# Onetism/LightFieldMicroscopy_PC-bzip2

Measured on AMD Instinct MI355X. Metric: uint16 Mpixel/s encode (predictor->bzip2) at 1/2/4/8 GPUs; ratio parity, higher is better.
Workload: dtype u16

## Files before the change

### include/lfm/lfm_hip.h

```cpp
#ifndef LFM_HIP_H
#define LFM_HIP_H

#include <stdint.h>
#include <stddef.h>

#ifdef __cplusplus
extern "C" {
#endif

enum lfm_hip_status {
    LFM_HIP_OK = 0,
    LFM_HIP_EINVAL = 1,
    LFM_HIP_ERUNTIME = 2,
    LFM_HIP_ENOTINV = 3,
    LFM_HIP_ENODEV = 4
};


int lfm_hip_predict(const uint16_t* d_in, const uint16_t* d_prev, uint16_t* d_out, int W, int H, int nframes,
                    int T, int family, int predictor, int video_bit, int z0, void* stream);

int lfm_hip_unpredict(const uint16_t* d_sym, const uint16_t* d_prev, uint16_t* d_out, int W, int H, int nframes,
                      int T, int family, int predictor, int video_bit, int z0, void* stream);
int lfm_hip_unpredict_async(const uint16_t* d_sym, const uint16_t* d_prev, uint16_t* d_out, int W, int H,
// ... 3 lines not shown
int lfm_hip_unpredict_path(int W, int H, int T);

int lfm_hip_predict_candidates(const uint16_t* d_frame, uint16_t* d_out7, int W, int H, int T, int family,
                               void* stream);

int lfm_hip_entropy2d(const uint16_t* d_cand, uint64_t npix, float* entropy, void* stream);

size_t lfm_hip_select_workspace_bytes(int W, int H);
int lfm_hip_select(const uint16_t* d_frame, int W, int H, int T, int family, float entropy[8], int* chosen,
                   void* d_workspace, void* stream);

size_t lfm_hip_bzip2_workspace_bytes(uint32_t count, uint32_t block_bytes);
size_t lfm_hip_bzip2_out_cap(uint32_t block_bytes);
int lfm_hip_bzip2_blocks(const void* d_img, const uint32_t dims[5], const uint32_t bs[5], uint32_t bpp,
                         uint32_t first, uint32_t count, uint32_t level, void* d_ws, size_t ws_bytes,
                         void* d_payload, uint64_t* h_sizes, uint32_t* h_flags, void* stream);
size_t lfm_hip_bzip2_workspace_bytes_multi(uint32_t count, uint32_t block_bytes, uint32_t level);
uint32_t lfm_hip_bzip2_max_count_multi(uint32_t block_bytes, uint32_t level);
int lfm_hip_bzip2_blocks_multi(const void* d_img, const uint32_t dims[5], const uint32_t bs[5], uint32_t bpp,
                               uint32_t first, uint32_t count, uint32_t level, void* d_ws, size_t ws_bytes,
                               void* d_payload, uint64_t* h_sizes, uint32_t* h_flags, void* stream);
uint64_t lfm_hip_bzip2_last_blocks(void);
void lfm_hip_bzip2_last_bwt_stats(uint32_t out[12]);
int lfm_hip_bzip2_last_stage_ms(float ms[5]);
void lfm_hip_bzip2_set_stage_hook(void (*fn)(void* ctx, int stage), void* ctx);

size_t lfm_hip_bunzip2_workspace_bytes(uint32_t count, uint32_t out_stride);
int lfm_hip_bunzip2_blocks(const void* d_payload, const uint64_t* h_offs, uint32_t count, void* d_out,
                           uint32_t out_stride, void* d_ws, size_t ws_bytes, uint32_t* h_lens, uint32_t* h_flags,
                           void* stream);
int lfm_hip_bunzip2_issue(const void* d_payload, const uint64_t* h_offs, uint32_t count, void* d_out,
                          uint32_t out_stride, void* d_ws, size_t ws_bytes, uint32_t* h_lens, uint32_t* h_flags,
                          void* stream);
uint32_t lfm_hip_bunzip2_max_parts(uint32_t out_stride, uint32_t level);
size_t lfm_hip_bunzip2_workspace_bytes_multi(uint32_t count, uint32_t out_stride, uint32_t level);
int lfm_hip_bunzip2_blocks_multi(const void* d_payload, const uint64_t* h_offs, uint32_t count, void* d_out,
                                 uint32_t out_stride, uint32_t level, void* d_ws, size_t ws_bytes, uint32_t* h_lens,
                                 uint32_t* h_flags, void* stream);
int lfm_hip_bunzip2_issue_multi(const void* d_payload, const uint64_t* h_offs, uint32_t count, void* d_out,
                                uint32_t out_stride, uint32_t level, void* d_ws, size_t ws_bytes, uint32_t* h_lens,
                                uint32_t* h_flags, void* stream);
int lfm_hip_bunzip2_set_periodic(int on);
int lfm_hip_bunzip2_get_periodic(void);

int lfm_hip_scatter_blocks(const void* d_blocks, uint32_t stride, uint32_t first, uint32_t count,
                           const uint32_t dims[5], const uint32_t bs[5], uint32_t bpp, void* d_img, void* stream);
// ... 16 lines not shown
```

### lightfieldmicroscopy_pc-bzip2_amd/csrc/lfm_bzip2.hip

```cpp
#include <hip/hip_runtime.h>
#include <rocprim/block/block_exchange.hpp>
#include <rocprim/block/block_sort.hpp>
#include <rocprim/device/device_radix_sort.hpp>
#include <rocprim/device/device_scan.hpp>
#include <rocprim/device/device_segmented_radix_sort.hpp>
#include <rocprim/device/device_select.hpp>
#include <rocprim/iterator/counting_iterator.hpp>
#include <algorithm>
#include <climits>
#include <cstdlib>
#include <cstdint>
#include <cstdio>
#include <cstring>
#include <mutex>
#include <type_traits>
#include <vector>
#include "lfm_bwt_types.h"
#include "lfm_bz_caps.h"
#include "lfm_hip.h"

#ifndef LFM_BWT_FORCE_FULL
#define LFM_BWT_FORCE_FULL 0
#endif

// ... 1012 lines not shown
            continue;
        }
        uint32_t* sv = B.sa + slot;
        bool ok = true;
        for (uint32_t x = 1; x < g && ok; ++x) {
            const uint32_t vx = sv[x];
            uint32_t y = x;
            while (y > 0) {
                const int cmp = tie_cmp(T, n, sv[y - 1] & kIdxMask, vx & kIdxMask);
                if (cmp == 0) {
                    ok = false;
                    break;
                }
                if (cmp < 0) break;
                sv[y] = sv[y - 1];
                --y;
            }
            sv[y] = vx;
        }
        if (!ok) atomicAdd(unres, 1u);
    }
}

template <int TH, int IPT>
__device__ __forceinline__ void chunk_load(const Batch& B, uint32_t cb, uint32_t m, uint32_t t, uint64_t (&k)[IPT],
                                           uint32_t (&v)[IPT])
{
    const uint32_t s = cb / B.cap, n = B.n[s];
    const uint8_t* T = B.T + (size_t)s * B.cap;
#pragma unroll
    for (int q = 0; q < IPT; ++q) v[q] = B.vals_a[cb + min(q * TH + t, m ? m - 1u : 0u)];
    uint32_t d[IPT][3];
#pragma unroll
    for (int q = 0; q < IPT; ++q) {
        const uint32_t i = v[q] & kIdxMask;
        const uint32_t* w = (const uint32_t*)(T + ((i + 8u <= n ? i : 0u) & ~3u));
        d[q][0] = w[0];
        d[q][1] = w[1];
        d[q][2] = w[2];
    }
#pragma unroll
    for (int q = 0; q < IPT; ++q) {
        const uint32_t j = q * TH + t, i = v[q] & kIdxMask;
        if (j >= m) {
            k[q] = ~0ull;
            v[q] = 0u;
        } else if (i + 8u <= n) {
            const uint32_t sh = (i & 3u) * 8u;
            const uint64_t x = (uint64_t)d[q][0] | ((uint64_t)d[q][1] << 32);
            k[q] = __builtin_bswap64(sh ? (x >> sh) | ((uint64_t)d[q][2] << (64u - sh)) : x);
        } else {
            k[q] = rot_key8_fast(T, n, i);
        }
    }
}

template <int TH, int IPT>
__global__ __launch_bounds__(TH) void bwt_chunk_sort(Batch B, const uint32_t* __restrict__ cbp,
                                                     const uint32_t* __restrict__ cep, uint32_t nch, uint32_t per)
{
    const uint32_t c = per ? (blockIdx.x & 7u) * per + (blockIdx.x >> 3) : blockIdx.x;
    if (c >= nch) return;
    static_assert(IPT == 2 || IPT == 4 || IPT == 8, "flags are packed 2, 4 or 8 per thread");
    using Sort = rocprim::block_sort<uint64_t, TH, IPT, uint32_t, rocprim::block_sort_algorithm::merge_sort>;
    using ExK = rocprim::block_exchange<uint64_t, TH, IPT>;
    using ExV = rocprim::block_exchange<uint32_t, TH, IPT>;
    constexpr uint32_t NI = TH * IPT;
    struct Xch {
        uint64_t first[TH], last[TH];
        uint32_t sv[NI];
        uint8_t fl[NI];
    };
    __shared__ union alignas(16) {
        typename Sort::storage_type s;
        typename ExK::storage_type ek;
        typename ExV::storage_type ev;
        Xch x;
    } sm;
    const uint32_t cb = cbp[c], ce = cep[c], m = ce - cb, t = threadIdx.x;
    uint64_t k[IPT];
    uint32_t v[IPT];
    chunk_load<TH, IPT>(B, cb, m, t, k, v);
    ExK().striped_to_blocked(k, k, sm.ek);
    __syncthreads();
    ExV().striped_to_blocked(v, v, sm.ev);
    __syncthreads();
    Sort().sort(k, v, sm.s, m);
    __syncthreads();
    sm.x.first[t] = k[0];
    sm.x.last[t] = k[IPT - 1];
    __syncthreads();
    const uint64_t kprev = t ? sm.x.last[t - 1] : 0ull, knext = t + 1 < (uint32_t)TH ? sm.x.first[t + 1] : 0ull;
    uint32_t nt = 0;
    uint64_t fpack = 0;
#pragma unroll
    for (int q = 0; q < IPT; ++q) {
        const uint32_t pos = t * IPT + q;
        const uint64_t lo = q ? k[q - 1] : kprev, hi = q + 1 < IPT ? k[q + 1] : knext;
        const bool f = pos < m && ((pos > 0 && lo == k[q]) || (pos + 1 < m && hi == k[q]));
        nt += f ? 1u : 0u;
        fpack |= (uint64_t)(f ? 1u : 0u) << (8 * q);
    }
    if constexpr (IPT == 2) {
        *(uint2*)&sm.x.sv[t * IPT] = make_uint2(v[0], v[1]);
        *(uint16_t*)&sm.x.fl[t * IPT] = (uint16_t)fpack;
    } else {
#pragma unroll
        for (int q = 0; q < IPT; q += 4) *(uint4*)&sm.x.sv[t * IPT + q] = make_uint4(v[q], v[q + 1], v[q + 2], v[q + 3]);
        if constexpr (IPT == 8) *(uint64_t*)&sm.x.fl[t * IPT] = fpack;
        else *(uint32_t*)&sm.x.fl[t * IPT] = (uint32_t)fpack;
    }
    __syncthreads();
    for (uint32_t j = t; j < m; j += TH) {
        B.sa[cb + j] = sm.x.sv[j];
        B.uflag[cb + j] = sm.x.fl[j];
    }
    if (__any(nt)) {
        for (int d = 32; d > 0; d >>= 1) nt += __shfl_xor(nt, d);
        if ((threadIdx.x & 63) == 0 && nt) atomicAdd(&B.done[cb / B.cap], nt);
    }
}

__device__ __forceinline__ uint64_t rot_key8(const Batch& B, uint32_t s, uint32_t i)
{
    const uint32_t n = B.n[s];
    const uint8_t* T = B.T + (size_t)s * B.cap;
    uint64_t k = 0;
    uint32_t j = i;
#pragma unroll
    for (int q = 0; q < 8; ++q) {
        k = (k << 8) | T[j];
        j = j + 1 == n ? 0u : j + 1;
    }
    return k;
}

__device__ __forceinline__ uint8_t tied_flag(const uint64_t* __restrict__ K, uint32_t cb, uint32_t ce, uint32_t j,
                                             uint64_t k)
// ... 238 lines not shown
__global__ __launch_bounds__(256) void bwt_comp_rank(Batch B, const uint32_t* __restrict__ cnt_p,
                                                     const uint32_t* __restrict__ hvs)
{
    const uint32_t cnt = *cnt_p;
    for (uint32_t c = blockIdx.x * blockDim.x + threadIdx.x; c < cnt; c += gridDim.x * blockDim.x) {
        const uint32_t head_slot = hvs[c];
        const uint32_t s = head_slot / B.cap;
        const size_t o = (size_t)s * B.cap;
        B.rank[o + (B.vals_b[c] & kIdxMask)] = (uint32_t)(head_slot - o);
        const bool head = c == 0 || B.keys_b[c] != B.keys_b[c - 1];
        const bool next_head = c + 1 >= cnt || B.keys_b[c + 1] != B.keys_b[c];
        B.uflag[c] = (head && next_head) ? 0 : 1;
    }
}

__global__ __launch_bounds__(256) void bwt_flag_periodic(Batch B, const uint32_t* __restrict__ cl,
                                                         const uint32_t* __restrict__ cnt_p)
{
    const uint32_t cnt = *cnt_p;
    for (uint32_t c = blockIdx.x * blockDim.x + threadIdx.x; c < cnt; c += gridDim.x * blockDim.x)
        atomicOr(&B.flags[cl[c] / B.cap], kFlagHost);
}

__device__ __forceinline__ void make_u2s(const Batch& B, uint32_t s, uint8_t* u2s, uint32_t lane, uint32_t* nin_out)
{
    uint32_t inu[8], nin = 0;
#pragma unroll
    for (int q = 0; q < 8; ++q) {
        inu[q] = B.inuse[s * 8 + q];
        nin += __popc(inu[q]);
    }
    for (uint32_t c = lane; c < 256; c += 64) {
        uint32_t below = 0;
        for (uint32_t q = 0; q < (c >> 5); ++q) below += __popc(inu[q]);
        below += __popc(inu[c >> 5] & ((1u << (c & 31)) - 1u));
        u2s[c] = (uint8_t)below;
    }
    *nin_out = nin;
}

constexpr uint32_t kIndPend = 0xFFFFFFFFu;
constexpr uint32_t kIndIdx = 0xFFFFFu;
constexpr uint32_t kIndPlaced = 1u << 23;
constexpr uint32_t kPlaceChunk = 2048;

__global__ __launch_bounds__(256) void bwt_place_sorted(Batch B, uint32_t chunks)
{
    __shared__ uint32_t tq[256], cs[256], cl[256], s0[256];
    __shared__ uint32_t cb[256];
    __shared__ uint8_t u2s[256];
    const uint32_t t = threadIdx.x, k = blockIdx.x >> 3;
    const uint32_t s = (blockIdx.x & 7u) + 8u * (k / chunks), base = (k % chunks) * kPlaceChunk;
    if (s >= B.nstreams || (B.flags[s] & kFlagHost)) return;
    const uint32_t n = B.n[s], ns = B.nsub[s], mode = B.bwt_mode[s];
    if (base >= n) return;
    const bool rev = mode == kModeSortA;
    if (t < 64) {
        uint32_t nin;
        make_u2s(B, s, u2s, t, &nin);
    }
    {
        const uint32_t* it = B.itab + (size_t)s * 1024;
        const uint32_t u = rev ? 255u - t : t;
        tq[t] = it[t];
        cs[t] = it[256 + t];
        cl[t] = it[512 + t];
        s0[t] = it[768 + t];
        cb[t] = it[256 + u] + it[512 + u] + (rev ? B.abcnt[(size_t)s * 512 + t] - 1u : 0u);
    }
    __syncthreads();
    const size_t o = (size_t)s * B.cap;
    const uint8_t* T = B.T + o;
    uint8_t* LL = (uint8_t*)B.mtfv + o;
    uint2* E = B.ent + o;
    constexpr int K = kPlaceChunk / 256;
    uint32_t v[K], w0[K], w1[K];
#pragma unroll
    for (int q = 0; q < K; ++q) v[q] = B.sa[o + min(base + q * 256 + t, ns ? ns - 1 : 0u)];
#pragma unroll
    for (int q = 0; q < K; ++q) {
        const uint32_t i = v[q] & kIdxMask, a = i >= 4 ? i - 4 : 0u;
        const uint32_t* w = (const uint32_t*)(T + (a & ~3u));
        w0[q] = w[0];
        w1[q] = w[1];
    }
#pragma unroll
    for (int q = 0; q < K; ++q) {
        const uint32_t j = base + q * 256 + t;
        if (j >= ns) break;
        const uint32_t i = v[q] & kIdxMask;
        uint32_t x;
        uint32_t c;
        if (i >= 4) {
            const uint32_t sh = ((i - 4) & 3u) * 8u;
            const uint64_t d = (uint64_t)w0[q] | ((uint64_t)w1[q] << 32);
            x = (uint32_t)(d >> sh);
            c = (uint32_t)(d >> (sh + 32)) & 0xFFu;
        } else {
            x = 0;
            for (uint32_t r = 1; r <= 4; ++r) x |= (uint32_t)T[(i + 4 * n - r) % n] << (32 - 8 * r);
            c = T[i];
        }
        const uint32_t r = j - s0[c], qq = tq[c] + r;
        LL[qq] = u2s[v[q] >> 24];
        if (i == 0) B.orig_ptr[s] = qq;
        if (mode != kModeFull)
            E[rev ? cb[c] - r : cb[c] + r] =
                make_uint2(v[q] | (3u << 20),
                           ((x >> 16) & 0xFFu) | (((x >> 8) & 0xFFu) << 8) | ((x & 0xFFu) << 16) | (c << 24));
    }
    if (mode == kModeFull) return;
    const uint32_t end = base + kPlaceChunk;
    uint32_t lo = 0, hi = 255;
    while (lo < hi) {
        const uint32_t mid = (lo + hi + 1) >> 1;
        if (cs[mid] <= base) lo = mid;
        else hi = mid - 1;
    }
    for (uint32_t u = lo; u < 256 && cs[u] < end; ++u)
        for (uint32_t q = max(cs[u], base) + t; q < min(cs[u] + cl[u], end); q += 256) E[q] = make_uint2(kIndPend, 0u);
}

constexpr uint32_t kIndSlices = 8;
constexpr uint32_t kIndBlock = 64 * kIndSlices;
constexpr int kIndStepSlices = 4;
constexpr uint32_t kIndRing = 2 * kIndBlock;

__device__ __forceinline__ void glds16(const void* g, const void* lds)
{
    const uint32_t m0 = __builtin_amdgcn_readfirstlane(
        (uint32_t)(size_t)(const __attribute__((address_space(3))) void*)lds);
    asm volatile("s_mov_b32 m0, %0\n\ts_nop 0\n\tglobal_load_lds_dwordx4 %1, off sc1" ::"s"(m0), "v"(g) : "memory", "m0");
}

__device__ __forceinline__ void vm_drain() { asm volatile("s_waitcnt vmcnt(0)" ::: "memory"); }

__global__ __launch_bounds__(64) void bwt_induce(Batch B)
{
    __shared__ uint32_t head[256], hlim[256];
    __shared__ uint32_t chead[256], clim[256];
    __shared__ uint2 ring[kIndRing];
    __shared__ __attribute__((aligned(16))) uint2 stg[kIndBlock];
    __shared__ uint8_t u2s[256];
// ... 1621 lines not shown
    float last_ms[5] = {};
    bool valid = false;
    ~StageEvents()
    {
        for (hipEvent_t e : ev)
            if (e) (void)hipEventDestroy(e);
    }
    bool ready(int d)
    {
        if (dev == d) return true;
        for (hipEvent_t& e : ev) {
            if (e) (void)hipEventDestroy(e);
            e = nullptr;
            if (hipEventCreate(&e) != hipSuccess) return false;
        }
        dev = d;
        return true;
    }
};
thread_local StageEvents t_stage;
thread_local void (*t_hook)(void*, int) = nullptr;
thread_local void* t_hook_ctx = nullptr;
thread_local uint64_t t_last_blocks = 0;
thread_local uint32_t t_last_bwt[12] = {};

size_t prim_tmp_bytes(uint32_t count, uint32_t cap)
{
    const size_t N = (size_t)count * cap;
    uint64_t* k = nullptr;
    uint32_t* v = nullptr;
    uint8_t* f = nullptr;
    size_t tmp = 0, q = 0;
    const size_t max_seg = (size_t)count * (cap / kBigCap + 1);
    (void)rocprim::segmented_radix_sort_pairs(nullptr, q, k, k, v, v, (unsigned)N, (unsigned)max_seg, v, v, 0,
                                              64 - kBucketBits);
    tmp = std::max(tmp, q);
    (void)rocprim::radix_sort_pairs(nullptr, q, k, k, v, v, (unsigned)N, 0, 64);
    tmp = std::max(tmp, q);

    (void)rocprim::select(nullptr, q, rocprim::counting_iterator<uint32_t>(0), f, v, v, N);
    tmp = std::max(tmp, q);
    (void)rocprim::select(nullptr, q, v, f, v, v, N);
    tmp = std::max(tmp, q);
    (void)rocprim::inclusive_scan(nullptr, q, v, v, N, rocprim::maximum<uint32_t>());
    tmp = std::max(tmp, q);
    return tmp;
}

struct Scratch {
    uint64_t* offs;
    uint32_t* cnt;
    void* tmp;
    size_t tmp_bytes;
};

struct BwtStats {
    uint32_t chunks[4] = {};
    uint32_t first_ties = 0;
    uint32_t left_runs = 0;
    uint32_t text_rounds = 0;
    uint32_t restarted = 0;
    uint32_t rank_form = 0;
    uint32_t doubling_rounds = 0;
    uint32_t flag_periodic = 0;
};

size_t layout(uint8_t* base, uint32_t streams, uint32_t block_bytes, uint32_t level, Batch& B, Scratch& S)
{
    B.parts = level ? max_parts(block_bytes, level) : 1u;
    const uint32_t count = streams * B.parts;
    B.nstreams = count;
    B.raw_cap = (uint32_t)align_up(block_bytes, 16);
    B.cap = rle_cap(block_bytes);
    B.out_cap = out_cap(block_bytes);
    B.sel_cap = sel_cap(block_bytes);
    B.full_cap = B.cap;
    if (B.parts > 1) {
        const uint32_t part_max = 100000u * level - 19u + 5u;
        B.cap = std::min(B.cap, (uint32_t)align_up((size_t)part_max + 64, 256));
        B.out_cap = std::min(B.out_cap, out_cap(part_max));
        B.sel_cap = (uint32_t)align_up(B.cap / kGSize + 8, 64);
    }
    B.jcap = B.parts * B.out_cap;
    B.pay_cap = out_cap(block_bytes);
    const size_t n = count, N = n * B.cap;
    size_t off = 0;
    auto take = [&](auto*& p, size_t bytes) {
// ... 47 lines not shown
struct TieRounds {
    hipStream_t st;
    size_t N;
    uint32_t* cnt;
    void* tmp;
    size_t tmp_bytes;
    uint32_t* cl;
    uint32_t* cl_next;
    uint32_t covered;
    bool none_left;
    BwtStats stats;
    uint64_t* gk;

    hipError_t read_count(uint32_t* out, size_t bytes = 4)
    {
        hipError_t e = hipMemcpyAsync(out, cnt, bytes, hipMemcpyDeviceToHost, st);
        return e != hipSuccess ? e : hipStreamSynchronize(st);
    }
};

uint32_t list_grid(uint32_t cnt) { return std::min<uint32_t>(4096, (cnt + 255) / 256); }

template <int TH, int IPT>
void chunk_sorts(const Batch& B, const ChunkLists& CL, int cls, uint32_t nc, hipStream_t st)
{
    const uint32_t per = (nc + 7) / 8;
    if (nc) hipLaunchKernelGGL((bwt_chunk_sort<TH, IPT>), dim3(8 * per), dim3(TH), 0, st, B, CL.b[cls], CL.e[cls], nc, per);
}

hipError_t first_round(const Batch& B, TieRounds& W)
{
    hipStream_t st = W.st;
    const uint32_t count = B.nstreams;
    hipError_t e;
    ChunkLists CL;
    const size_t q = W.N / 4;
    for (int c = 0; c < 4; ++c) {
        CL.b[c] = B.cl0 + c * q;
        CL.e[c] = B.cl1 + c * q;
    }
    CL.cnt = W.cnt;
    CL.cnt3 = W.cnt + 5;
    uint32_t nch[6] = {0, 0, 0, 0, 0, 0};
    if ((e = hipMemsetAsync(W.cnt, 0, 32, st)) != hipSuccess ||
        (e = hipMemsetAsync(B.done, 0, (size_t)count * 4, st)) != hipSuccess)
        return e;
    hipLaunchKernelGGL(bwt_bucket<kBucketBits>, dim3(count), dim3(kBucketThreads), 0, st, B, CL);
    if ((e = hipGetLastError()) != hipSuccess || (e = W.read_count(nch, 24)) != hipSuccess) return e;
    W.stats.chunks[0] = nch[5];
    W.stats.chunks[1] = nch[0];
    W.stats.chunks[2] = nch[1];
    W.stats.chunks[3] = nch[2];
    W.stats.first_ties = W.stats.left_runs = W.stats.text_rounds = 0;
    chunk_sorts<kTinyCap / kCsItems, kCsItems>(B, CL, 3, nch[5], st);
    chunk_sorts<kCsThreads, kCsItems>(B, CL, 0, nch[0], st);
    chunk_sorts<kBigThreads, kBigItems>(B, CL, 1, nch[1], st);
    if (nch[2]) {
        hipLaunchKernelGGL(bwt_chunk_keys, dim3(nch[2]), dim3(256), 0, st, B, CL.b[2], CL.e[2]);
        e = rocprim::segmented_radix_sort_pairs(W.tmp, W.tmp_bytes, B.keys_a, B.keys_b, B.vals_a, B.sa,
                                                (unsigned)W.N, nch[2], CL.b[2], CL.e[2], 0, 64 - kBucketBits, st);
        if (e == hipSuccess)
            hipLaunchKernelGGL(bwt_chunk_flags, dim3(nch[2]), dim3(256), 0, st, B, CL.b[2], CL.e[2]);
    }
    if ((e = hipGetLastError()) != hipSuccess) return e;
    W.cl = B.cl0;
    W.cl_next = B.cl1;
    hipLaunchKernelGGL(tie_offsets, dim3(1), dim3(1024), 0, st, B, W.cnt);
    hipLaunchKernelGGL(tie_compact, dim3(count), dim3(256), 0, st, B, B.cl0);
    hipLaunchKernelGGL(tie_runs_direct, dim3(1024), dim3(256), 0, st, B, B.cl0, W.cnt, W.cnt + 7);
    W.covered = kKeyBytes;
    W.none_left = false;
    return hipGetLastError();
}

hipError_t text_rounds(const Batch& B, TieRounds& W)
{
    hipStream_t st = W.st;
    uint32_t* bnd = (uint32_t*)B.mtfv;
    for (int r = 0; r < kTextRounds; ++r) {
        uint32_t c8[8] = {};
        hipError_t e = W.read_count(c8, r == 0 ? 32 : 4);
        if (e != hipSuccess) return e;
        const uint32_t cnt = c8[0];
        if (r == 0) {
            W.stats.first_ties = cnt;
            W.stats.left_runs = c8[7];
        }
        if (cnt == 0 || (r == 0 && c8[7] == 0)) {
            W.none_left = true;
            break;
        }
        if ((size_t)cnt * 4 > W.N) break;
// ... 168 lines not shown
    Scratch S{};
    if (ws_bytes < layout((uint8_t*)d_ws, streams, raw_cap, multi ? level : 0u, B, S)) return LFM_HIP_EINVAL;
    count = B.nstreams;
    if ((size_t)count * B.cap >= (1ull << 32)) return LFM_HIP_EINVAL;
    const bool parts = B.parts > 1;

    hipError_t e = hipSuccess;
    auto ok = [&]() { return (e = hipGetLastError()) == hipSuccess; };
    const bool from_img = ((uintptr_t)d_img & 15) == 0 && (bs[0] * bpp) % 16 == 0 && (dims[0] * bpp) % 16 == 0 &&
                          ((dims[0] % bs[0]) * bpp) % 16 == 0;
    mark(0);
    if (!from_img) hipLaunchKernelGGL(gather_blocks, dim3(64, streams), dim3(256), 0, st, B);
    if (!parts) {
        if (from_img) hipLaunchKernelGGL((rle1_crc<true, false>), dim3(count), dim3(kRleThreads), 0, st, B);
        else hipLaunchKernelGGL((rle1_crc<false, false>), dim3(count), dim3(kRleThreads), 0, st, B);
    } else {
        if (from_img) hipLaunchKernelGGL((rle1_crc<true, true>), dim3(streams), dim3(kRleThreads), 0, st, B);
        else hipLaunchKernelGGL((rle1_crc<false, true>), dim3(streams), dim3(kRleThreads), 0, st, B);
        hipLaunchKernelGGL(place_parts, dim3(16, count), dim3(256), 0, st, B);
    }
    if (!ok()) return LFM_HIP_ERUNTIME;
    mark(1);
    BwtStats bwt_stats;
    if (bwt_sort(B, S, st, &bwt_stats) != hipSuccess) return LFM_HIP_ERUNTIME;
    {
        const uint32_t v[12] = {bwt_stats.chunks[0], bwt_stats.chunks[1], bwt_stats.chunks[2], bwt_stats.chunks[3],
                                bwt_stats.first_ties, bwt_stats.left_runs, bwt_stats.text_rounds, bwt_stats.restarted,
                                bwt_stats.rank_form, bwt_stats.doubling_rounds, bwt_stats.flag_periodic, 0u};
        std::copy(v, v + 12, t_last_bwt);
    }
    if (!B.it_full) {
        B.ent = (uint2*)B.keys_a;
        const uint32_t chunks = (B.cap + kPlaceChunk - 1) / kPlaceChunk;
        hipLaunchKernelGGL(bwt_place_sorted, dim3(8 * chunks * ((count + 7) / 8)), dim3(256), 0, st, B, chunks);
        hipLaunchKernelGGL(bwt_induce, dim3(count), dim3(64), 0, st, B);
        if (!ok()) return LFM_HIP_ERUNTIME;
    }
    mark(2);
    if (t_hook) t_hook(t_hook_ctx, 1);
    {
        const uint32_t nseg_max = (B.cap + kSeg - 1) / kSeg;
        int32_t* seg_last = (int32_t*)B.keys_a;
        const dim3 g((nseg_max + 3) / 4, count);
        if (B.it_full) hipLaunchKernelGGL(mtf_last<false>, g, dim3(256), 0, st, B, nseg_max, seg_last);
        else hipLaunchKernelGGL(mtf_last<true>, g, dim3(256), 0, st, B, nseg_max, seg_last);
        hipLaunchKernelGGL(mtf_prefix, dim3(count), dim3(256), 0, st, B, nseg_max, seg_last);
        hipLaunchKernelGGL(mtf_win, g, dim3(256), 0, st, B, nseg_max, (const int32_t*)seg_last);
        hipLaunchKernelGGL(rle2, dim3(count), dim3(kRle2Threads), 0, st, B);
    }
    uint32_t nwide = 0;
    if (!ok() || hipMemcpyAsync(&nwide, B.wide_cnt, 4, hipMemcpyDeviceToHost, st) != hipSuccess ||
        hipStreamSynchronize(st) != hipSuccess || nwide > count)
        return LFM_HIP_ERUNTIME;
    mark(3);
    if (t_hook) t_hook(t_hook_ctx, 2);
    hipLaunchKernelGGL(huff_init, dim3(count), dim3(64), 0, st, B);
    static thread_local struct TablesEvent {
// ... 73 lines not shown

extern "C" int lfm_hip_bzip2_blocks_multi(const void* d_img, const uint32_t dims[5], const uint32_t bs[5],
                                          uint32_t bpp, uint32_t first, uint32_t count, uint32_t level, void* d_ws,
                                          size_t ws_bytes, void* d_payload, uint64_t* h_sizes, uint32_t* h_flags,
                                          void* stream)
{
    return bzip2_blocks(d_img, dims, bs, bpp, first, count, level, d_ws, ws_bytes, d_payload, h_sizes, h_flags, stream,
                        true);
}

extern "C" void lfm_hip_bzip2_set_stage_hook(void (*fn)(void*, int), void* ctx)
{
    t_hook = fn;
    t_hook_ctx = ctx;
}

extern "C" uint64_t lfm_hip_bzip2_last_blocks(void) { return t_last_blocks; }

extern "C" void lfm_hip_bzip2_last_bwt_stats(uint32_t out[12])
{
    if (out) std::copy(t_last_bwt, t_last_bwt + 12, out);
}

extern "C" int lfm_hip_bzip2_last_stage_ms(float ms[5])
{
    if (!ms || !t_stage.valid) return 3;
    for (int i = 0; i < 5; ++i) ms[i] = t_stage.last_ms[i];
    return 0;
}
```

### lightfieldmicroscopy_pc-bzip2_amd/lfm/__init__.py

```python
import ctypes
import os

import numpy as np

try:
    import torch
    _HAVE_TORCH = True
except Exception:
    _HAVE_TORCH = False

PKG_DIR = os.path.dirname(os.path.dirname(os.path.abspath(__file__)))
LIB_PATH = os.environ.get("LFM_LIB") or os.path.join(PKG_DIR, "liblfm.so")

FAMILIES = {"tiles": 0, "angle_and_space": 0, "angle": 1, "space": 2}
DTYPES = {np.dtype(np.uint8): 0, np.dtype(np.uint16): 1, np.dtype(np.uint32): 2, np.dtype(np.uint64): 3,
          np.dtype(np.int8): 4, np.dtype(np.int16): 5, np.dtype(np.int32): 6, np.dtype(np.int64): 7,
          np.dtype(np.float32): 8, np.dtype(np.float64): 9}
NP_OF = {v: k for k, v in DTYPES.items()}

EXPORTS = [
    "writeKLBstack", "writeKLBstackSlices", "readKLBheader", "readKLBstack", "readKLBstackInPlace",
    "readKLBroiInPlace",
    "lfm_set_family", "lfm_get_family", "lfm_version", "lfm_api_version", "writeLFMstack_c", "readLFMstack_c",
    "lfm_encoder_create", "lfm_encoder_destroy", "lfm_encoder_encode", "lfm_encoder_encode_slab",
    "lfm_merge_slabs", "lfm_free", "lfm_decode_memory", "lfm_decode_memory_roi", "lfm_set_devices", "lfm_get_devices", "lfm_default_devices",
    "lfm_encoder_encode_multi", "lfm_release_encoders", "lfm_slab_info", "lfm_place_slab", "lfm_encoder_submit",
    "lfm_encoder_submit_select", "lfm_encoder_wait", "lfm_decode_memory_device", "lfm_decode_memory_roi_device",
    "lfm_set_decode_devices", "lfm_get_decode_devices", "lfm_default_decode_devices", "lfm_release_decoders",
    "lfm_decode_shard_plan", "lfm_decode_memory_multi", "lfm_decode_memory_multi_device",
    "lfm_set_bzip2_multiblock", "lfm_get_bzip2_multiblock", "lfm_encoder_stream_counts",
    "lfm_set_bunzip2_multiblock", "lfm_get_bunzip2_multiblock",
    "lfm_set_bunzip2_periodic", "lfm_get_bunzip2_periodic",
    "lfm_hip_predict", "lfm_hip_unpredict", "lfm_hip_unpredict_async", "lfm_hip_unpredict_check",
    "lfm_hip_unpredict_path",
    "lfm_hip_predict_candidates", "lfm_hip_entropy2d", "lfm_hip_select_workspace_bytes", "lfm_hip_select",
    "lfm_hip_synth", "lfm_hip_device_count", "lfm_hip_force_generic", "lfm_hip_bzip2_workspace_bytes", "lfm_hip_bzip2_out_cap",
    "lfm_hip_bzip2_blocks", "lfm_hip_bzip2_last_stage_ms", "lfm_hip_bunzip2_workspace_bytes", "lfm_hip_bunzip2_blocks", "lfm_hip_scatter_blocks",
    "lfm_hip_crop_region", "lfm_hip_bzip2_workspace_bytes_multi", "lfm_hip_bzip2_max_count_multi",
    "lfm_hip_bzip2_blocks_multi", "lfm_hip_bzip2_last_blocks", "lfm_hip_bzip2_last_bwt_stats",
    "lfm_hip_bunzip2_max_parts", "lfm_hip_bunzip2_workspace_bytes_multi", "lfm_hip_bunzip2_blocks_multi",
    "lfm_hip_bunzip2_issue_multi", "lfm_hip_bunzip2_set_periodic", "lfm_hip_bunzip2_get_periodic",
]


class LfmError(RuntimeError):
    pass


class EncodeStats(ctypes.Structure):
    _fields_ = [("total_ms", ctypes.c_double), ("h2d_ms", ctypes.c_double), ("select_ms", ctypes.c_double),
                ("predict_ms", ctypes.c_double), ("d2h_ms", ctypes.c_double), ("compress_ms", ctypes.c_double),
                ("chosen", ctypes.c_int), ("header_version", ctypes.c_int), ("entropy", ctypes.c_float * 8),
                ("out_bytes", ctypes.c_uint64), ("bz_stage_ms", ctypes.c_double * 5), ("bz_in_bytes", ctypes.c_uint64)]
    BZ_STAGES = ("rle1", "bwt", "mtf", "huffman", "emit")

    def as_dict(self):
        d = {f: getattr(self, f) for f, _ in self._fields_ if f not in ("entropy", "bz_stage_ms")}
        d["entropy"] = list(self.entropy)
        d["bz_stage_ms"] = dict(zip(self.BZ_STAGES, list(self.bz_stage_ms)))
        return d


# ... 90 lines not shown
    L.lfm_decode_memory_roi.argtypes = [vp, ctypes.c_uint64, u32p, u32p, vp, ctypes.c_uint64, ctypes.c_int]
    L.lfm_hip_predict.argtypes = [vp, vp, vp] + [ctypes.c_int] * 8 + [vp]
    L.lfm_hip_unpredict.argtypes = [vp, vp, vp] + [ctypes.c_int] * 8 + [vp]
    L.lfm_hip_unpredict_async.argtypes = [vp, vp, vp] + [ctypes.c_int] * 8 + [vp, vp]
    L.lfm_hip_unpredict_check.argtypes = [ctypes.c_int]
    L.lfm_hip_predict_candidates.argtypes = [vp, vp] + [ctypes.c_int] * 4 + [vp]
    L.lfm_hip_entropy2d.argtypes = [vp, ctypes.c_uint64, f32p, vp]
    L.lfm_hip_bzip2_workspace_bytes.argtypes = [ctypes.c_uint32, ctypes.c_uint32]
    L.lfm_hip_bzip2_workspace_bytes.restype = ctypes.c_size_t
    L.lfm_hip_bzip2_out_cap.argtypes = [ctypes.c_uint32]
    L.lfm_hip_bzip2_out_cap.restype = ctypes.c_size_t
    L.lfm_hip_bzip2_blocks.argtypes = [vp, u32p, u32p, ctypes.c_uint32, ctypes.c_uint32, ctypes.c_uint32,
                                       ctypes.c_uint32, vp, ctypes.c_size_t, vp,
                                       ctypes.POINTER(ctypes.c_uint64), ctypes.POINTER(ctypes.c_uint32), vp]
    L.lfm_hip_bzip2_workspace_bytes_multi.argtypes = [ctypes.c_uint32] * 3
    L.lfm_hip_bzip2_workspace_bytes_multi.restype = ctypes.c_size_t
    L.lfm_hip_bzip2_max_count_multi.argtypes = [ctypes.c_uint32] * 2
    L.lfm_hip_bzip2_max_count_multi.restype = ctypes.c_uint32
    L.lfm_hip_bzip2_blocks_multi.argtypes = L.lfm_hip_bzip2_blocks.argtypes
    L.lfm_hip_bzip2_last_blocks.argtypes = []
    L.lfm_hip_bzip2_last_blocks.restype = ctypes.c_uint64
    L.lfm_hip_bzip2_last_bwt_stats.argtypes = [u32p]
    L.lfm_hip_bzip2_last_bwt_stats.restype = None
    L.lfm_set_bzip2_multiblock.argtypes = [ctypes.c_int]
    L.lfm_get_bzip2_multiblock.argtypes = []
    L.lfm_encoder_stream_counts.argtypes = [vp] + [ctypes.POINTER(ctypes.c_uint64)] * 3
    L.lfm_hip_bunzip2_workspace_bytes.argtypes = [ctypes.c_uint32, ctypes.c_uint32]
    L.lfm_hip_bunzip2_workspace_bytes.restype = ctypes.c_size_t
    L.lfm_hip_bunzip2_blocks.argtypes = [vp, ctypes.POINTER(ctypes.c_uint64), ctypes.c_uint32, vp, ctypes.c_uint32,
                                         vp, ctypes.c_size_t, u32p, u32p, vp]
    L.lfm_hip_bunzip2_max_parts.argtypes = [ctypes.c_uint32] * 2
    L.lfm_hip_bunzip2_max_parts.restype = ctypes.c_uint32
    L.lfm_hip_bunzip2_workspace_bytes_multi.argtypes = [ctypes.c_uint32] * 3
    L.lfm_hip_bunzip2_workspace_bytes_multi.restype = ctypes.c_size_t
    L.lfm_hip_bunzip2_blocks_multi.argtypes = [vp, ctypes.POINTER(ctypes.c_uint64), ctypes.c_uint32, vp,
                                               ctypes.c_uint32, ctypes.c_uint32, vp, ctypes.c_size_t, u32p, u32p, vp]
    L.lfm_set_bunzip2_multiblock.argtypes = [ctypes.c_int]
    L.lfm_get_bunzip2_multiblock.argtypes = []
    L.lfm_set_bunzip2_periodic.argtypes = [ctypes.c_int]
    L.lfm_get_bunzip2_periodic.argtypes = []
    L.lfm_hip_scatter_blocks.argtypes = [vp, ctypes.c_uint32, ctypes.c_uint32, ctypes.c_uint32, u32p, u32p,
                                         ctypes.c_uint32, vp, vp]
    L.lfm_hip_select_workspace_bytes.restype = ctypes.c_size_t
    L.lfm_hip_select_workspace_bytes.argtypes = [ctypes.c_int, ctypes.c_int]
    L.lfm_hip_select.argtypes = [vp, ctypes.c_int, ctypes.c_int, ctypes.c_int, ctypes.c_int, f32p,
                                 ctypes.POINTER(ctypes.c_int), vp, vp]
# ... 634 lines not shown
              ws.data_ptr(), ws_bytes, pay.data_ptr(), sizes, flags, _stream(stream)),
           "lfm_hip_bzip2_blocks_multi" if multi else "lfm_hip_bzip2_blocks")
    host = pay[:int(sum(sizes))].cpu().numpy().tobytes()
    out, o = [], 0
    for i in range(count):
        if flags[i]:
            out.append(None)
        else:
            out.append(host[o:o + sizes[i]])
            o += sizes[i]
    return out, list(flags)


BWT_STATS = ("chunks_tiny", "chunks_small", "chunks_big", "chunks_segmented", "first_ties", "left_runs",
             "text_rounds", "restarted", "rank_form", "doubling_rounds", "flag_periodic")


def bzip2_last_bwt_stats():
    out = (ctypes.c_uint32 * 12)()
    lib().lfm_hip_bzip2_last_bwt_stats(out)
    return dict(zip(BWT_STATS, list(out)))


def set_bunzip2_multiblock(on):
    return bool(lib().lfm_set_bunzip2_multiblock(1 if on else 0))


def get_bunzip2_multiblock():
    return bool(lib().lfm_get_bunzip2_multiblock())


def set_bunzip2_periodic(on):
    return bool(lib().lfm_set_bunzip2_periodic(1 if on else 0))


def get_bunzip2_periodic():
    return bool(lib().lfm_get_bunzip2_periodic())


def bunzip2_max_parts(out_stride, level):
    return int(lib().lfm_hip_bunzip2_max_parts(out_stride, level))


def bunzip2_device(streams, out_stride, device="cuda", stream=None, multi=False, level=None):
    count = len(streams)
    offs = np.zeros(count + 1, dtype=np.uint64)
# ... 32 lines not shown
```

Measured before the change: 16910.

## Fuse BWT sorted-slot placement into chunk sort kernels when no segmented sorts

When all first-round chunks are handled by the in-block chunk sorts (no segmented radix sort) and no further tie rounds are needed, the placement of L-column symbols and induce entries happens inside bwt_chunk_sort rather than in a separate bwt_place_sorted pass. Tied slots are placed afterwards by a new bwt_place_tied kernel that uses global tables, and bwt_pend_live marks the pending entries. This avoids a full re-read of the suffix array and text in a separate kernel. The cost is extra shared memory and registers in the sort kernels, plus added complexity in choosing the placement path at runtime, which is exposed through a new query function.

```diff
diff --git a/include/lfm/lfm_hip.h b/include/lfm/lfm_hip.h
--- a/include/lfm/lfm_hip.h
+++ b/include/lfm/lfm_hip.h
@@ -49,6 +49,7 @@
                                void* d_payload, uint64_t* h_sizes, uint32_t* h_flags, void* stream);
 uint64_t lfm_hip_bzip2_last_blocks(void);
 void lfm_hip_bzip2_last_bwt_stats(uint32_t out[12]);
+uint32_t lfm_hip_bzip2_last_place_path(void);
 int lfm_hip_bzip2_last_stage_ms(float ms[5]);
 void lfm_hip_bzip2_set_stage_hook(void (*fn)(void* ctx, int stage), void* ctx);
 
diff --git a/lightfieldmicroscopy_pc-bzip2_amd/csrc/lfm_bzip2.hip b/lightfieldmicroscopy_pc-bzip2_amd/csrc/lfm_bzip2.hip
--- a/lightfieldmicroscopy_pc-bzip2_amd/csrc/lfm_bzip2.hip
+++ b/lightfieldmicroscopy_pc-bzip2_amd/csrc/lfm_bzip2.hip
@@ -1058,6 +1058,104 @@
     }
 }
 
+__device__ __forceinline__ void make_u2s(const Batch& B, uint32_t s, uint8_t* u2s, uint32_t lane, uint32_t* nin_out)
+{
+    uint32_t inu[8], nin = 0;
+#pragma unroll
+    for (int q = 0; q < 8; ++q) {
+        inu[q] = B.inuse[s * 8 + q];
+        nin += __popc(inu[q]);
+    }
+    for (uint32_t c = lane; c < 256; c += 64) {
+        uint32_t below = 0;
+        for (uint32_t q = 0; q < (c >> 5); ++q) below += __popc(inu[q]);
+        below += __popc(inu[c >> 5] & ((1u << (c & 31)) - 1u));
+        u2s[c] = (uint8_t)below;
+    }
+    *nin_out = nin;
+}
+
+constexpr uint32_t kIndPend = 0xFFFFFFFFu;
+constexpr uint32_t kIndIdx = 0xFFFFFu;
+constexpr uint32_t kIndPlaced = 1u << 23;
+
+struct PlaceTabs {
+    uint32_t tq_[256], s0_[256], cb_[256];
+    uint8_t u2s_[256];
+    __device__ __forceinline__ uint32_t tq(uint32_t c) const { return tq_[c]; }
+    __device__ __forceinline__ uint32_t s0(uint32_t c) const { return s0_[c]; }
+    __device__ __forceinline__ uint32_t cb(uint32_t c) const { return cb_[c]; }
+    __device__ __forceinline__ uint32_t sym(uint32_t b) const { return u2s_[b]; }
+};
+
+__device__ __forceinline__ uint32_t place_cb(const uint32_t* __restrict__ it, const uint32_t* __restrict__ ab, bool rev,
+                                            uint32_t c)
+{
+    const uint32_t u = rev ? 255u - c : c;
+    return it[256 + u] + it[512 + u] + (rev ? ab[c] - 1u : 0u);
+}
+
+__device__ __forceinline__ void place_tabs_load(const Batch& B, uint32_t s, uint32_t mode, PlaceTabs& P, uint32_t t)
+{
+    if (t < 64) {
+        uint32_t nin;
+        make_u2s(B, s, P.u2s_, t, &nin);
+    }
+    if (t < 256) {
+        const uint32_t* it = B.itab + (size_t)s * 1024;
+        P.tq_[t] = it[t];
+        P.s0_[t] = it[768 + t];
+        P.cb_[t] = place_cb(it, B.abcnt + (size_t)s * 512, mode == kModeSortA, t);
+    }
+}
+
+struct PlaceTabsGlobal {
+    const uint32_t* it;
+    const uint32_t* ab;
+    const uint32_t* inuse;
+    bool rev;
+    __device__ __forceinline__ uint32_t tq(uint32_t c) const { return it[c]; }
+    __device__ __forceinline__ uint32_t s0(uint32_t c) const { return it[768 + c]; }
+    __device__ __forceinline__ uint32_t cb(uint32_t c) const { return place_cb(it, ab, rev, c); }
+    __device__ __forceinline__ uint32_t sym(uint32_t b) const
+    {
+        uint32_t below = __popc(inuse[b >> 5] & ((1u << (b & 31)) - 1u));
+        for (uint32_t q = 0; q < (b >> 5); ++q) below += __popc(inuse[q]);
+        return below;
+    }
+};
+
+__device__ __forceinline__ const uint32_t* place_text_at(const uint8_t* __restrict__ T, uint32_t i)
+{
+    return (const uint32_t*)(T + ((i >= 4 ? i - 4 : 0u) & ~3u));
+}
+__device__ __forceinline__ void place_text(const uint8_t* __restrict__ T, uint32_t n, uint32_t i, uint32_t w0, uint32_t w1,
+                                           uint32_t& x, uint32_t& c)
+{
+    if (i >= 4) {
+        const uint32_t sh = ((i - 4) & 3u) * 8u;
+        const uint64_t d = (uint64_t)w0 | ((uint64_t)w1 << 32);
+        x = (uint32_t)(d >> sh);
+        c = (uint32_t)(d >> (sh + 32)) & 0xFFu;
+    } else {
+        x = 0;
+        for (uint32_t r = 1; r <= 4; ++r) x |= (uint32_t)T[(i + 4 * n - r) % n] << (32 - 8 * r);
+        c = T[i];
+    }
+}
+
+template <class Tabs>
+__device__ __forceinline__ void place_slot(const Tabs& P, uint32_t mode, uint32_t j, uint32_t v, uint32_t x, uint32_t c,
+                                           uint8_t* __restrict__ LL, uint2* __restrict__ E, uint32_t* __restrict__ orig_ptr)
+{
+    const uint32_t r = j - P.s0(c), qq = P.tq(c) + r;
+    LL[qq] = (uint8_t)P.sym(v >> 24);
+    if ((v & kIdxMask) == 0) *orig_ptr = qq;
+    if (mode != kModeFull)
+        E[mode == kModeSortA ? P.cb(c) - r : P.cb(c) + r] =
+            make_uint2(v | (3u << 20), ((x >> 16) & 0xFFu) | (((x >> 8) & 0xFFu) << 8) | ((x & 0xFFu) << 16) | (c << 24));
+}
+
 template <int TH, int IPT>
 __device__ __forceinline__ void chunk_load(const Batch& B, uint32_t cb, uint32_t m, uint32_t t, uint64_t (&k)[IPT],
                                            uint32_t (&v)[IPT])
@@ -1091,7 +1189,7 @@
     }
 }
 
-template <int TH, int IPT>
+template <int TH, int IPT, bool PLACE>
 __global__ __launch_bounds__(TH) void bwt_chunk_sort(Batch B, const uint32_t* __restrict__ cbp,
                                                      const uint32_t* __restrict__ cep, uint32_t nch, uint32_t per)
 {
@@ -1113,7 +1211,10 @@
         typename ExV::storage_type ev;
         Xch x;
     } sm;
+    __shared__ std::conditional_t<PLACE, PlaceTabs, char> P;
     const uint32_t cb = cbp[c], ce = cep[c], m = ce - cb, t = threadIdx.x;
+    const uint32_t s = cb / B.cap, mode = PLACE ? B.bwt_mode[s] : 0u;
+    if constexpr (PLACE) place_tabs_load(B, s, mode, P, t);
     uint64_t k[IPT];
     uint32_t v[IPT];
     chunk_load<TH, IPT>(B, cb, m, t, k, v);
@@ -1147,9 +1248,33 @@
         else *(uint32_t*)&sm.x.fl[t * IPT] = (uint32_t)fpack;
     }
     __syncthreads();
+    [[maybe_unused]] const uint8_t* T = B.T + (size_t)s * B.cap;
+    [[maybe_unused]] uint32_t w0[IPT], w1[IPT];
+    if constexpr (PLACE) {
+#pragma unroll
+        for (int q = 0; q < IPT; ++q) {
+            const uint32_t* w = place_text_at(T, v[q] & kIdxMask);
+            w0[q] = w[0];
+            w1[q] = w[1];
+        }
+    }
     for (uint32_t j = t; j < m; j += TH) {
         B.sa[cb + j] = sm.x.sv[j];
         B.uflag[cb + j] = sm.x.fl[j];
+    }
+    if constexpr (PLACE) {
+        const size_t o = (size_t)s * B.cap;
+        const uint32_t n = B.n[s], j0 = cb - (uint32_t)o + t * IPT;
+        uint8_t* LL = (uint8_t*)B.mtfv + o;
+        uint2* E = B.ent + o;
+#pragma unroll
+        for (int q = 0; q < IPT; ++q) {
+            if (t * IPT + q < m) {
+                uint32_t x, ci;
+                place_text(T, n, v[q] & kIdxMask, w0[q], w1[q], x, ci);
+                place_slot(P, mode, j0 + q, v[q], x, (uint32_t)(k[q] >> 56), LL, E, B.orig_ptr + s);
+            }
+        }
     }
     if (__any(nt)) {
         for (int d = 32; d > 0; d >>= 1) nt += __shfl_xor(nt, d);
@@ -1434,52 +1559,20 @@
         atomicOr(&B.flags[cl[c] / B.cap], kFlagHost);
 }
 
-__device__ __forceinline__ void make_u2s(const Batch& B, uint32_t s, uint8_t* u2s, uint32_t lane, uint32_t* nin_out)
-{
-    uint32_t inu[8], nin = 0;
-#pragma unroll
-    for (int q = 0; q < 8; ++q) {
-        inu[q] = B.inuse[s * 8 + q];
-        nin += __popc(inu[q]);
-    }
-    for (uint32_t c = lane; c < 256; c += 64) {
-        uint32_t below = 0;
-        for (uint32_t q = 0; q < (c >> 5); ++q) below += __popc(inu[q]);
-        below += __popc(inu[c >> 5] & ((1u << (c & 31)) - 1u));
-        u2s[c] = (uint8_t)below;
-    }
-    *nin_out = nin;
-}
-
-constexpr uint32_t kIndPend = 0xFFFFFFFFu;
-constexpr uint32_t kIndIdx = 0xFFFFFu;
-constexpr uint32_t kIndPlaced = 1u << 23;
 constexpr uint32_t kPlaceChunk = 2048;
 
 __global__ __launch_bounds__(256) void bwt_place_sorted(Batch B, uint32_t chunks)
 {
-    __shared__ uint32_t tq[256], cs[256], cl[256], s0[256];
-    __shared__ uint32_t cb[256];
-    __shared__ uint8_t u2s[256];
+    __shared__ PlaceTabs P;
+    __shared__ uint32_t cs[256], cl[256];
     const uint32_t t = threadIdx.x, k = blockIdx.x >> 3;
     const uint32_t s = (blockIdx.x & 7u) + 8u * (k / chunks), base = (k % chunks) * kPlaceChunk;
     if (s >= B.nstreams || (B.flags[s] & kFlagHost)) return;
     const uint32_t n = B.n[s], ns = B.nsub[s], mode = B.bwt_mode[s];
     if (base >= n) return;
-    const bool rev = mode == kModeSortA;
-    if (t < 64) {
-        uint32_t nin;
-        make_u2s(B, s, u2s, t, &nin);
-    }
-    {
-        const uint32_t* it = B.itab + (size_t)s * 1024;
-        const uint32_t u = rev ? 255u - t : t;
-        tq[t] = it[t];
-        cs[t] = it[256 + t];
-        cl[t] = it[512 + t];
-        s0[t] = it[768 + t];
-        cb[t] = it[256 + u] + it[512 + u] + (rev ? B.abcnt[(size_t)s * 512 + t] - 1u : 0u);
-    }
+    place_tabs_load(B, s, mode, P, t);
+    cs[t] = B.itab[(size_t)s * 1024 + 256 + t];
+    cl[t] = B.itab[(size_t)s * 1024 + 512 + t];
     __syncthreads();
     const size_t o = (size_t)s * B.cap;
     const uint8_t* T = B.T + o;
@@ -1491,8 +1584,7 @@
     for (int q = 0; q < K; ++q) v[q] = B.sa[o + min(base + q * 256 + t, ns ? ns - 1 : 0u)];
 #pragma unroll
     for (int q = 0; q < K; ++q) {
-        const uint32_t i = v[q] & kIdxMask, a = i >= 4 ? i - 4 : 0u;
-        const uint32_t* w = (const uint32_t*)(T + (a & ~3u));
+        const uint32_t* w = place_text_at(T, v[q] & kIdxMask);
         w0[q] = w[0];
         w1[q] = w[1];
     }
@@ -1500,26 +1592,9 @@
     for (int q = 0; q < K; ++q) {
         const uint32_t j = base + q * 256 + t;
         if (j >= ns) break;
-        const uint32_t i = v[q] & kIdxMask;
-        uint32_t x;
-        uint32_t c;
-        if (i >= 4) {
-            const uint32_t sh = ((i - 4) & 3u) * 8u;
-            const uint64_t d = (uint64_t)w0[q] | ((uint64_t)w1[q] << 32);
-            x = (uint32_t)(d >> sh);
-            c = (uint32_t)(d >> (sh + 32)) & 0xFFu;
-        } else {
-            x = 0;
-            for (uint32_t r = 1; r <= 4; ++r) x |= (uint32_t)T[(i + 4 * n - r) % n] << (32 - 8 * r);
-            c = T[i];
-        }
-        const uint32_t r = j - s0[c], qq = tq[c] + r;
-        LL[qq] = u2s[v[q] >> 24];
-        if (i == 0) B.orig_ptr[s] = qq;
-        if (mode != kModeFull)
-            E[rev ? cb[c] - r : cb[c] + r] =
-                make_uint2(v[q] | (3u << 20),
-                           ((x >> 16) & 0xFFu) | (((x >> 8) & 0xFFu) << 8) | ((x & 0xFFu) << 16) | (c << 24));
+        uint32_t x, c;
+        place_text(T, n, v[q] & kIdxMask, w0[q], w1[q], x, c);
+        place_slot(P, mode, j, v[q], x, c, LL, E, B.orig_ptr + s);
     }
     if (mode == kModeFull) return;
     const uint32_t end = base + kPlaceChunk;
@@ -1531,6 +1606,40 @@
     }
     for (uint32_t u = lo; u < 256 && cs[u] < end; ++u)
         for (uint32_t q = max(cs[u], base) + t; q < min(cs[u] + cl[u], end); q += 256) E[q] = make_uint2(kIndPend, 0u);
+}
+
+__global__ __launch_bounds__(256) void bwt_pend_live(Batch B)
+{
+    const uint32_t s = blockIdx.x, lane = threadIdx.x & 63;
+    if (B.flags[s] & kFlagHost) return;
+    const uint32_t n = B.n[s];
+    if (n == 0 || B.bwt_mode[s] == kModeFull) return;
+    __shared__ uint32_t c0[256], c1[256];
+    const uint32_t* it = B.itab + (size_t)s * 1024;
+    uint2* E = B.ent + (size_t)s * B.cap;
+    c0[threadIdx.x] = it[256 + threadIdx.x];
+    c1[threadIdx.x] = min(it[256 + threadIdx.x] + it[512 + threadIdx.x], n);
+    __syncthreads();
+    for (uint32_t u = threadIdx.x >> 6; u < 256; u += 4)
+        for (uint32_t q = c0[u] + lane; q < c1[u]; q += 64) E[q] = make_uint2(kIndPend, 0u);
+}
+
+__global__ __launch_bounds__(256) void bwt_place_tied(Batch B, const uint32_t* __restrict__ cl,
+                                                      const uint32_t* __restrict__ cnt_p)
+{
+    const uint32_t cnt = *cnt_p;
+    for (uint32_t c = blockIdx.x * blockDim.x + threadIdx.x; c < cnt; c += gridDim.x * blockDim.x) {
+        const uint32_t slot = cl[c];
+        const uint32_t s = slot / B.cap, n = B.n[s], mode = B.bwt_mode[s];
+        const size_t o = (size_t)s * B.cap;
+        const uint8_t* T = B.T + o;
+        const uint32_t v = B.sa[slot], i = v & kIdxMask;
+        const uint32_t* w = place_text_at(T, i);
+        uint32_t x, ch;
+        place_text(T, n, i, w[0], w[1], x, ch);
+        const PlaceTabsGlobal P{B.itab + (size_t)s * 1024, B.abcnt + (size_t)s * 512, B.inuse + s * 8, mode == kModeSortA};
+        place_slot(P, mode, slot - (uint32_t)o, v, x, ch, (uint8_t*)B.mtfv + o, B.ent + o, B.orig_ptr + s);
+    }
 }
 
 constexpr uint32_t kIndSlices = 8;
@@ -3198,6 +3307,7 @@
 thread_local void (*t_hook)(void*, int) = nullptr;
 thread_local void* t_hook_ctx = nullptr;
 thread_local uint64_t t_last_blocks = 0;
+thread_local uint32_t t_last_place = 0;
 thread_local uint32_t t_last_bwt[12] = {};
 
 size_t prim_tmp_bytes(uint32_t count, uint32_t cap)
@@ -3239,6 +3349,12 @@
     uint32_t rank_form = 0;
     uint32_t doubling_rounds = 0;
     uint32_t flag_periodic = 0;
+    bool fused_sorts = false;
+
+    uint32_t place_path(bool it_full) const
+    {
+        return it_full ? 0u : (fused_sorts && left_runs == 0 && text_rounds == 0) ? 1u : 2u;
+    }
 };
 
 size_t layout(uint8_t* base, uint32_t streams, uint32_t block_bytes, uint32_t level, Batch& B, Scratch& S)
@@ -3332,10 +3448,12 @@
 uint32_t list_grid(uint32_t cnt) { return std::min<uint32_t>(4096, (cnt + 255) / 256); }
 
 template <int TH, int IPT>
-void chunk_sorts(const Batch& B, const ChunkLists& CL, int cls, uint32_t nc, hipStream_t st)
+void chunk_sorts(const Batch& B, const ChunkLists& CL, int cls, uint32_t nc, bool place, hipStream_t st)
 {
     const uint32_t per = (nc + 7) / 8;
-    if (nc) hipLaunchKernelGGL((bwt_chunk_sort<TH, IPT>), dim3(8 * per), dim3(TH), 0, st, B, CL.b[cls], CL.e[cls], nc, per);
+    if (!nc) return;
+    if (place) hipLaunchKernelGGL((bwt_chunk_sort<TH, IPT, true>), dim3(8 * per), dim3(TH), 0, st, B, CL.b[cls], CL.e[cls], nc, per);
+    else hipLaunchKernelGGL((bwt_chunk_sort<TH, IPT, false>), dim3(8 * per), dim3(TH), 0, st, B, CL.b[cls], CL.e[cls], nc, per);
 }
 
 hipError_t first_round(const Batch& B, TieRounds& W)
@@ -3362,9 +3480,11 @@
     W.stats.chunks[2] = nch[1];
     W.stats.chunks[3] = nch[2];
     W.stats.first_ties = W.stats.left_runs = W.stats.text_rounds = 0;
-    chunk_sorts<kTinyCap / kCsItems, kCsItems>(B, CL, 3, nch[5], st);
-    chunk_sorts<kCsThreads, kCsItems>(B, CL, 0, nch[0], st);
-    chunk_sorts<kBigThreads, kBigItems>(B, CL, 1, nch[1], st);
+    const bool fused = !B.it_full && nch[2] == 0;
+    W.stats.fused_sorts = fused;
+    chunk_sorts<kTinyCap / kCsItems, kCsItems>(B, CL, 3, nch[5], fused, st);
+    chunk_sorts<kCsThreads, kCsItems>(B, CL, 0, nch[0], fused, st);
+    chunk_sorts<kBigThreads, kBigItems>(B, CL, 1, nch[1], fused, st);
     if (nch[2]) {
         hipLaunchKernelGGL(bwt_chunk_keys, dim3(nch[2]), dim3(256), 0, st, B, CL.b[2], CL.e[2]);
         e = rocprim::segmented_radix_sort_pairs(W.tmp, W.tmp_bytes, B.keys_a, B.keys_b, B.vals_a, B.sa,
@@ -3378,6 +3498,10 @@
     hipLaunchKernelGGL(tie_offsets, dim3(1), dim3(1024), 0, st, B, W.cnt);
     hipLaunchKernelGGL(tie_compact, dim3(count), dim3(256), 0, st, B, B.cl0);
     hipLaunchKernelGGL(tie_runs_direct, dim3(1024), dim3(256), 0, st, B, B.cl0, W.cnt, W.cnt + 7);
+    if (fused) {
+        hipLaunchKernelGGL(bwt_place_tied, dim3(256), dim3(256), 0, st, B, B.cl0, W.cnt);
+        hipLaunchKernelGGL(bwt_pend_live, dim3(count), dim3(256), 0, st, B);
+    }
     W.covered = kKeyBytes;
     W.none_left = false;
     return hipGetLastError();
@@ -3592,7 +3716,9 @@
     if (!ok()) return LFM_HIP_ERUNTIME;
     mark(1);
     BwtStats bwt_stats;
+    B.ent = (uint2*)B.keys_a;
     if (bwt_sort(B, S, st, &bwt_stats) != hipSuccess) return LFM_HIP_ERUNTIME;
+    t_last_place = bwt_stats.place_path(B.it_full != 0);
     {
         const uint32_t v[12] = {bwt_stats.chunks[0], bwt_stats.chunks[1], bwt_stats.chunks[2], bwt_stats.chunks[3],
                                 bwt_stats.first_ties, bwt_stats.left_runs, bwt_stats.text_rounds, bwt_stats.restarted,
@@ -3600,9 +3726,9 @@
         std::copy(v, v + 12, t_last_bwt);
     }
     if (!B.it_full) {
-        B.ent = (uint2*)B.keys_a;
         const uint32_t chunks = (B.cap + kPlaceChunk - 1) / kPlaceChunk;
-        hipLaunchKernelGGL(bwt_place_sorted, dim3(8 * chunks * ((count + 7) / 8)), dim3(256), 0, st, B, chunks);
+        if (t_last_place == 2)
+            hipLaunchKernelGGL(bwt_place_sorted, dim3(8 * chunks * ((count + 7) / 8)), dim3(256), 0, st, B, chunks);
         hipLaunchKernelGGL(bwt_induce, dim3(count), dim3(64), 0, st, B);
         if (!ok()) return LFM_HIP_ERUNTIME;
     }
@@ -3722,6 +3848,8 @@
     if (out) std::copy(t_last_bwt, t_last_bwt + 12, out);
 }
 
+extern "C" uint32_t lfm_hip_bzip2_last_place_path(void) { return t_last_place; }
+
 extern "C" int lfm_hip_bzip2_last_stage_ms(float ms[5])
 {
     if (!ms || !t_stage.valid) return 3;
diff --git a/lightfieldmicroscopy_pc-bzip2_amd/lfm/__init__.py b/lightfieldmicroscopy_pc-bzip2_amd/lfm/__init__.py
--- a/lightfieldmicroscopy_pc-bzip2_amd/lfm/__init__.py
+++ b/lightfieldmicroscopy_pc-bzip2_amd/lfm/__init__.py
@@ -38,6 +38,7 @@
     "lfm_hip_bzip2_blocks", "lfm_hip_bzip2_last_stage_ms", "lfm_hip_bunzip2_workspace_bytes", "lfm_hip_bunzip2_blocks", "lfm_hip_scatter_blocks",
     "lfm_hip_crop_region", "lfm_hip_bzip2_workspace_bytes_multi", "lfm_hip_bzip2_max_count_multi",
     "lfm_hip_bzip2_blocks_multi", "lfm_hip_bzip2_last_blocks", "lfm_hip_bzip2_last_bwt_stats",
+    "lfm_hip_bzip2_last_place_path",
     "lfm_hip_bunzip2_max_parts", "lfm_hip_bunzip2_workspace_bytes_multi", "lfm_hip_bunzip2_blocks_multi",
     "lfm_hip_bunzip2_issue_multi", "lfm_hip_bunzip2_set_periodic", "lfm_hip_bunzip2_get_periodic",
 ]
@@ -174,6 +175,8 @@
     L.lfm_hip_bzip2_last_blocks.restype = ctypes.c_uint64
     L.lfm_hip_bzip2_last_bwt_stats.argtypes = [u32p]
     L.lfm_hip_bzip2_last_bwt_stats.restype = None
+    L.lfm_hip_bzip2_last_place_path.argtypes = []
+    L.lfm_hip_bzip2_last_place_path.restype = ctypes.c_uint32
     L.lfm_set_bzip2_multiblock.argtypes = [ctypes.c_int]
     L.lfm_get_bzip2_multiblock.argtypes = []
     L.lfm_encoder_stream_counts.argtypes = [vp] + [ctypes.POINTER(ctypes.c_uint64)] * 3
@@ -854,6 +857,10 @@
     return dict(zip(BWT_STATS, list(out)))
 
 
+def bzip2_last_place_path():
+    return int(lib().lfm_hip_bzip2_last_place_path())
+
+
 def set_bunzip2_multiblock(on):
     return bool(lib().lfm_set_bunzip2_multiblock(1 if on else 0))
 
```

Result: faster. 17850, median of 6 (+5.6%).
